# angeladai/sgnn

Measured on AMD Instinct MI355X. Metric: TSDF blocks/sec fwd+bwd (64^3@5% occ, bs32), higher is better.
Workload: dtype f32

## Files before the change

sgnn_amd/csrc/linear.hip:

```cpp
#include "common.h"

#define LIN_MAX_OUT 4
#define LIN_MAX_BLOCKS 512

template <int CIN, int VEC>
__device__ __forceinline__ void load_row(const float *__restrict__ p, float (&v)[CIN]) {
  if constexpr (VEC == 4) {
#pragma unroll
    for (int t = 0; t < CIN / 4; ++t) {
      const float4 q = reinterpret_cast<const float4 *>(p)[t];
      v[4 * t] = q.x; v[4 * t + 1] = q.y; v[4 * t + 2] = q.z; v[4 * t + 3] = q.w;
    }
  } else {
#pragma unroll
    for (int t = 0; t < CIN; ++t) v[t] = p[t];
  }
}

struct LinW {
  const float *w[LIN_MAX_OUT];
  const float *b[LIN_MAX_OUT];
};
struct LinG {
  float *dw[LIN_MAX_OUT];
  float *db[LIN_MAX_OUT];
};

template <int CIN, int COUT>
__global__ __launch_bounds__(256) void k_linear_fwd(const float *__restrict__ x, int64_t n, LinW p,
                                                   float *__restrict__ y, const int64_t *n_dev) {
  __shared__ float ws[COUT * CIN + COUT];
  n = sgnn_dyn_n(n, n_dev);
  for (int e = threadIdx.x; e < COUT * CIN; e += 256) ws[e] = p.w[e / CIN][e % CIN];
  if (threadIdx.x < COUT) ws[COUT * CIN + threadIdx.x] = p.b[threadIdx.x] ? p.b[threadIdx.x][0] : 0.f;
  __syncthreads();
  const int64_t stride = (int64_t)gridDim.x * 256;
  for (int64_t r = (int64_t)blockIdx.x * 256 + threadIdx.x; r < n; r += stride) {
    float v[CIN];
    load_row<CIN, (CIN % 4 == 0) ? 4 : 1>(x + r * CIN, v);
#pragma unroll
    for (int o = 0; o < COUT; ++o) {
      float acc = ws[COUT * CIN + o];
#pragma unroll
      for (int c = 0; c < CIN; ++c) acc = fmaf(v[c], ws[o * CIN + c], acc);
      y[r * COUT + o] = acc;
    }
  }
}

template <int CIN, int COUT>
__global__ __launch_bounds__(256) void k_linear_bwd(const float *__restrict__ x, const float *__restrict__ dy,
                                                   int64_t n, LinW p, float *dx, double *__restrict__ partial,
                                                   const int64_t *n_dev, const float *addend, int64_t ld_add) {
  constexpr int NV = COUT * CIN + COUT;
  n = sgnn_dyn_n(n, n_dev);
  __shared__ float ws[COUT * CIN];
  __shared__ float red[4][NV];
  for (int e = threadIdx.x; e < COUT * CIN; e += 256) ws[e] = p.w[e / CIN][e % CIN];
  __syncthreads();
  float acc[NV];
#pragma unroll
  for (int e = 0; e < NV; ++e) acc[e] = 0.f;
  const int64_t stride = (int64_t)gridDim.x * 256;
  for (int64_t r = (int64_t)blockIdx.x * 256 + threadIdx.x; r < n; r += stride) {
    float v[CIN], g[COUT];
    load_row<CIN, (CIN % 4 == 0) ? 4 : 1>(x + r * CIN, v);
#pragma unroll
    for (int o = 0; o < COUT; ++o) g[o] = dy[r * COUT + o];
#pragma unroll
    for (int o = 0; o < COUT; ++o) {
#pragma unroll
      for (int c = 0; c < CIN; ++c) acc[o * CIN + c] = fmaf(g[o], v[c], acc[o * CIN + c]);
      acc[COUT * CIN + o] += g[o];
    }
    if (dx) {
      float d[CIN];
#pragma unroll
      for (int c = 0; c < CIN; ++c) {
        float t = 0.f;
#pragma unroll
        for (int o = 0; o < COUT; ++o) t = fmaf(g[o], ws[o * CIN + c], t);
        d[c] = t;
      }
      if (addend) {
        float a[CIN];
        load_row<CIN, (CIN % 4 == 0) ? 4 : 1>(addend + r * ld_add, a);
#pragma unroll
        for (int c = 0; c < CIN; ++c) d[c] += a[c];
      }
      if constexpr (CIN % 4 == 0) {
#pragma unroll
        for (int t = 0; t < CIN / 4; ++t)
          reinterpret_cast<float4 *>(dx + r * CIN)[t] = make_float4(d[4 * t], d[4 * t + 1], d[4 * t + 2], d[4 * t + 3]);
      } else {
#pragma unroll
        for (int c = 0; c < CIN; ++c) dx[r * CIN + c] = d[c];
      }
    }
  }
  const int lane = threadIdx.x & 63, wave = threadIdx.x >> 6;
#pragma unroll
  for (int e = 0; e < NV; ++e) {
    float t = acc[e];
#pragma unroll
    for (int d = 32; d > 0; d >>= 1) t += __shfl_xor(t, d);
    if (lane == 0) red[wave][e] = t;
  }
  __syncthreads();
  for (int e = threadIdx.x; e < NV; e += 256)
    partial[(size_t)blockIdx.x * NV + e] = (double)red[0][e] + (double)red[1][e] + (double)red[2][e] + (double)red[3][e];
}

__global__ __launch_bounds__(256) void k_linear_finalize(const double *__restrict__ partial, int nblk, int nv,
                                                        int ncw, int cin, LinG g) {
  __shared__ double sh[256];
  const int e = blockIdx.x;
  double a = 0.0;
  for (int b = threadIdx.x; b < nblk; b += 256) a += partial[(size_t)b * nv + e];
  sh[threadIdx.x] = a;
  __syncthreads();
  for (int d = 128; d > 0; d >>= 1) {
    if (threadIdx.x < d) sh[threadIdx.x] += sh[threadIdx.x + d];
    __syncthreads();
  }
  if (threadIdx.x == 0) {
    if (e < ncw) {
      if (g.dw[e / cin]) g.dw[e / cin][e % cin] = (float)sh[0];
    } else if (g.db[e - ncw]) {
      g.db[e - ncw][0] = (float)sh[0];
    }
  }
}

static int lin_blocks(int64_t n) {
  int64_t b = (n + 255) / 256;
  if (b < 1) b = 1;
  if (b > LIN_MAX_BLOCKS) b = LIN_MAX_BLOCKS;
  return (int)b;
}

SGNN_EXPORT int64_t sgnn_linear_ws_bytes(int64_t n, int cin, int cout) {
  (void)n;
  return (int64_t)LIN_MAX_BLOCKS * (cin * cout + cout) * (int64_t)sizeof(double) + 256;
}

#define LIN_CASES(X) X(16, 1) X(16, 2) X(48, 1) X(48, 2) X(8, 1) X(8, 2) X(32, 1) X(32, 2) X(12, 2) X(4, 1)

static bool lin_shape_ok(int cin, int cout) {
#define X(CI, CO) if (cin == CI && cout == CO) return true;
  LIN_CASES(X)
#undef X
  return false;
}

int sgnn_linear_fwd_rows(const float *x, int64_t n, int cin, const float *const *w, const float *const *b, int cout,
                         float *y, sgnn_stream_t stream, const int64_t *n_dev) {
  SGNN_CHECK_ARG(n >= 0 && cin >= 1 && cout >= 1 && cout <= LIN_MAX_OUT);
  if (!lin_shape_ok(cin, cout)) {
    sgnn_set_error("sgnn_linear_fwd: unsupported head shape %d -> %d", cin, cout);
    return SGNN_EINVAL;
  }
  if (n == 0) return SGNN_OK;
  SGNN_CHECK_ARG(x && w && y);
  LinW p{};
  for (int o = 0; o < cout; ++o) {
    SGNN_CHECK_ARG(w[o]);
    p.w[o] = w[o];
    p.b[o] = b ? b[o] : nullptr;
  }
  hipStream_t s = (hipStream_t)stream;
  const int grid = sgnn_grid_for(n, 256, 2048);
  bool done = false;
#define X(CI, CO)                                                                                   \
  if (!done && cin == CI && cout == CO) {                                                           \
    SGNN_LAUNCH((k_linear_fwd<CI, CO>), dim3(grid), dim3(256), 0, s, x, n, p, y, n_dev);     \
    done = true;                                                                                    \
  }
  LIN_CASES(X)
#undef X
  if (!done) {
    sgnn_set_error("sgnn_linear_fwd: unsupported head shape %d -> %d", cin, cout);
    return SGNN_EINVAL;
  }
  SGNN_CHECK_LAUNCH();
  return SGNN_OK;
}

SGNN_EXPORT int sgnn_linear_fwd(const float *x, int64_t n, int cin, const float *w, const float *bias, int cout,
                                float *y, sgnn_stream_t stream) {
  SGNN_CHECK_ARG(cout >= 1 && cout <= LIN_MAX_OUT && cin >= 1);
  const float *wr[LIN_MAX_OUT] = {}, *br[LIN_MAX_OUT] = {};
  for (int o = 0; o < cout; ++o) {
    wr[o] = w ? w + (size_t)o * cin : nullptr;
    br[o] = bias ? bias + o : nullptr;
  }
  return sgnn_linear_fwd_rows(x, n, cin, wr, br, cout, y, stream);
}

int sgnn_linear_bwd_rows(const float *x, const float *dy, int64_t n, int cin, const float *const *w, int cout,
                         float *dx, float *const *dw, float *const *db, void *ws, int64_t ws_bytes,
                         sgnn_stream_t stream, const int64_t *n_dev, const float *addend, int64_t ld_add) {
  hipStream_t s = (hipStream_t)stream;
  SGNN_CHECK_ARG(n >= 0 && cin >= 1 && cout >= 1 && cout <= LIN_MAX_OUT && w);
  SGNN_CHECK_ARG(!addend || (dx && ld_add >= cin && (cin % 4 != 0 || (ld_add % 4 == 0 && ((uintptr_t)addend & 15) == 0))));
  if (!lin_shape_ok(cin, cout)) {
    sgnn_set_error("sgnn_linear_bwd: unsupported head shape %d -> %d", cin, cout);
    return SGNN_EINVAL;
  }
  if (n == 0) {
    for (int o = 0; o < cout; ++o) {
      if (dw && dw[o]) SGNN_HIP_TRY(hipMemsetAsync(dw[o], 0, (size_t)cin * sizeof(float), s));
      if (db && db[o]) SGNN_HIP_TRY(hipMemsetAsync(db[o], 0, sizeof(float), s));
    }
    return SGNN_OK;
  }
  SGNN_CHECK_ARG(x && dy);
  if (!ws || ws_bytes < sgnn_linear_ws_bytes(n, cin, cout)) {
    sgnn_set_error("sgnn_linear_bwd: workspace too small");
    return SGNN_ENOWS;
  }
  LinW p{};
  LinG g{};
  for (int o = 0; o < cout; ++o) {
    SGNN_CHECK_ARG(w[o]);
    p.w[o] = w[o];
    g.dw[o] = dw ? dw[o] : nullptr;
    g.db[o] = db ? db[o] : nullptr;
  }
  const int nblk = lin_blocks(n);
  const int nv = cin * cout + cout;
  bool done = false;
#define X(CI, CO)                                                                                          \
  if (!done && cin == CI && cout == CO) {                                                                  \
    SGNN_LAUNCH((k_linear_bwd<CI, CO>), dim3(nblk), dim3(256), 0, s, x, dy, n, p, dx, (double *)ws, n_dev, addend, ld_add); \
    done = true;                                                                                           \
  }
  LIN_CASES(X)
#undef X
  if (!done) {
    sgnn_set_error("sgnn_linear_bwd: unsupported head shape %d -> %d", cin, cout);
    return SGNN_EINVAL;
  }
  SGNN_LAUNCH(k_linear_finalize, dim3(nv), dim3(256), 0, s, (const double *)ws, nblk, nv, cin * cout, cin, g);
  SGNN_CHECK_LAUNCH();
  return SGNN_OK;
}

SGNN_EXPORT int sgnn_linear_bwd(const float *x, const float *dy, int64_t n, int cin, const float *w, int cout,
                                float *dx, float *dw, float *dbias, void *ws, int64_t ws_bytes,
                                sgnn_stream_t stream) {
  SGNN_CHECK_ARG(cout >= 1 && cout <= LIN_MAX_OUT && cin >= 1 && w);
  const float *wr[LIN_MAX_OUT] = {};
  float *dwr[LIN_MAX_OUT] = {}, *dbr[LIN_MAX_OUT] = {};
  for (int o = 0; o < cout; ++o) {
    wr[o] = w + (size_t)o * cin;
    dwr[o] = dw ? dw + (size_t)o * cin : nullptr;
    dbr[o] = dbias ? dbias + o : nullptr;
  }
  return sgnn_linear_bwd_rows(x, dy, n, cin, wr, cout, dx, dwr, dbr, ws, ws_bytes, stream);
}
```

sgnn_amd/csrc/loss.hip:

```cpp
#include "common.h"

#define LOSS_MAX_BLOCKS 512
#define UNK_ID_F (-1.0f)
#define UNK_THRESH_U8 2

struct LossArgs {
  const int64_t *locs;
  const float *vals;
  int vstride, occ_col, sdf_col;
  const float *tgt_occ;
  const float *tgt_sdf;
  const float *weights;
  const uint8_t *known;
  int d0, d1, d2;
  int64_t m;
  const int64_t *m_dev;
  int use_log;
  int mask_mode;
};

__device__ __forceinline__ float logt(float v) { return copysignf(logf(fabsf(v) + 1.0f), v) * (v != 0.f); }

__device__ __forceinline__ bool loss_site(const LossArgs &a, int64_t r, float &bce, float &l1, float &dbce, float &dl1) {
  const longlong2 p0 = reinterpret_cast<const longlong2 *>(a.locs)[2 * r];
  const longlong2 p1 = reinterpret_cast<const longlong2 *>(a.locs)[2 * r + 1];
  const int64_t fl = ((p1.y * a.d0 + p0.x) * a.d1 + p0.y) * a.d2 + p1.x;
  const float w = a.weights ? a.weights[fl] : 1.0f;
  float to = 0.f;
  bool keep = true;
  if (a.tgt_occ) to = a.tgt_occ[fl];
  if (a.mask_mode == 1) keep = (to != UNK_ID_F);
  if (a.mask_mode == 2) keep = a.known[fl] < UNK_THRESH_U8;
  if (a.mask_mode == 0 && to == UNK_ID_F) to = 0.f;
  bce = l1 = dbce = dl1 = 0.f;
  if (!keep) return false;
  if (a.occ_col >= 0) {
    const float x = a.vals[r * a.vstride + a.occ_col];
    const float t = fmaxf(to, 0.f);
    bce = w * (fmaxf(x, 0.f) - x * t + log1pf(expf(-fabsf(x))));
    dbce = w * (1.0f / (1.0f + expf(-x)) - t);
  }
  if (a.sdf_col >= 0) {
    const float p = a.vals[r * a.vstride + a.sdf_col];
    const float t = a.tgt_sdf[fl];
    const float d = a.use_log ? (logt(p) - logt(t)) : (p - t);
    l1 = w * fabsf(d);
    const float sg = (d > 0.f) ? 1.f : ((d < 0.f) ? -1.f : 0.f);
    dl1 = w * sg * (a.use_log ? 1.0f / (fabsf(p) + 1.0f) : 1.0f);
  }
  return true;
}

static int loss_blocks(int64_t m) {
  int64_t b = (m + 1023) / 1024;
  if (b < 1) b = 1;
  if (b > LOSS_MAX_BLOCKS) b = LOSS_MAX_BLOCKS;
  return (int)b;
}

static int fill_args(LossArgs &a, const int64_t *locs, const float *vals, int vstride, int occ_col, int sdf_col,
                     const float *tgt_occ, const float *tgt_sdf, const float *weights, const uint8_t *known, int d0,
                     int d1, int d2, int64_t m, int use_log, int mask_mode, const int64_t *m_dev) {
  if (!(m >= 0 && vstride >= 1 && occ_col < vstride && sdf_col < vstride && (occ_col >= 0 || sdf_col >= 0))) return -1;
  if (m > 0 && (!locs || !vals)) return -1;
  if (occ_col >= 0 && !tgt_occ) return -1;
  if (sdf_col >= 0 && !tgt_sdf) return -1;
  if (mask_mode == 1 && !tgt_occ) return -1;
  if (mask_mode == 2 && !known) return -1;
  if (mask_mode < 0 || mask_mode > 2) return -1;
  a = LossArgs{locs, vals, vstride, occ_col, sdf_col, tgt_occ, tgt_sdf, weights, known, d0, d1, d2, m, m_dev, use_log, mask_mode};
  return 0;
}

#define LOSS_MAX_LEVELS 5
struct LossMulti {
  LossArgs a[LOSS_MAX_LEVELS];
  float coef[2 * LOSS_MAX_LEVELS];
  int nblk[LOSS_MAX_LEVELS];
  int n;
};
struct LossOut {
  float *dvals[LOSS_MAX_LEVELS];
};

__global__ __launch_bounds__(256) void k_loss_partial(LossMulti m, double *__restrict__ partial) {
  __shared__ double sh[3][256];
  const int l = blockIdx.y;
  const LossArgs &a = m.a[l];
  if ((int)blockIdx.x >= m.nblk[l]) return;
  double s[3] = {0.0, 0.0, 0.0};
  const int64_t stride = (int64_t)m.nblk[l] * 256;
  const int64_t rows = sgnn_dyn_n(a.m, a.m_dev);
  for (int64_t r = (int64_t)blockIdx.x * 256 + threadIdx.x; r < rows; r += stride) {
    float bce, l1, db, dl;
    if (loss_site(a, r, bce, l1, db, dl)) {
      s[0] += (double)bce;
      s[1] += (double)l1;
      s[2] += 1.0;
    }
  }
  sgnn_block_sum256(sh, s);
  if (threadIdx.x < 3) partial[((size_t)l * LOSS_MAX_BLOCKS + blockIdx.x) * 3 + threadIdx.x] = sh[threadIdx.x][0];
}

__global__ __launch_bounds__(256) void k_loss_finalize(const double *__restrict__ partial, LossMulti m,
                                                      double *__restrict__ sums, float *__restrict__ out2s,
                                                      float *__restrict__ total, float *__restrict__ cur) {
  __shared__ double sh[3][256];
  for (int l = 0; l < m.n; ++l) {
    double s[3] = {0.0, 0.0, 0.0};
    for (int b = threadIdx.x; b < m.nblk[l]; b += 256)
      for (int c = 0; c < 3; ++c) s[c] += partial[((size_t)l * LOSS_MAX_BLOCKS + b) * 3 + c];
    sgnn_block_sum256(sh, s);
    if (threadIdx.x == 0) {
      sums[3 * l + 0] = sh[0][0];
      sums[3 * l + 1] = sh[1][0];
      sums[3 * l + 2] = sh[2][0];
      const bool empty = m.a[l].m_dev && *m.a[l].m_dev <= 0;
      out2s[2 * l] = empty ? 0.f : (float)(sh[0][0] / sh[2][0]);
      out2s[2 * l + 1] = empty ? 0.f : (float)(sh[1][0] / sh[2][0]);
    }
    __syncthreads();
  }
  if (threadIdx.x == 0) {
    float t = 0.f;
    for (int i = 0; i < 2 * m.n; ++i)
      if (m.coef[i] != 0.f) t += m.coef[i] * out2s[i];
    *total = t;
    for (int l = 0; l < m.n; ++l)
      cur[l] = (m.coef[2 * l] != 0.f ? out2s[2 * l] : 0.f) + (m.coef[2 * l + 1] != 0.f ? out2s[2 * l + 1] : 0.f);
  }
}

__global__ __launch_bounds__(256) void k_loss_bwd(LossMulti m, const double *__restrict__ sums,
                                                 const float *__restrict__ g, LossOut o) {
  const int l = blockIdx.y;
  const LossArgs &a = m.a[l];
  float *dvals = o.dvals[l];
  const double kept = sums[3 * l + 2];
  const float g0 = (float)((double)(g[0] * m.coef[2 * l]) / kept), g1 = (float)((double)(g[0] * m.coef[2 * l + 1]) / kept);
  const int64_t stride = (int64_t)gridDim.x * 256;
  const int64_t rows = sgnn_dyn_n(a.m, a.m_dev);
  for (int64_t r = (int64_t)blockIdx.x * 256 + threadIdx.x; r < rows; r += stride) {
    float bce, l1, db, dl;
    const bool keep = loss_site(a, r, bce, l1, db, dl);
    for (int c = 0; c < a.vstride; ++c) {
      float v = 0.f;
      if (keep && c == a.occ_col) v = g0 * db;
      if (keep && c == a.sdf_col) v = g1 * dl;
      dvals[r * a.vstride + c] = v;
    }
  }
}

SGNN_EXPORT int64_t sgnn_loss_multi_ws_bytes(void) {
  return (int64_t)LOSS_MAX_LEVELS * LOSS_MAX_BLOCKS * 3 * sizeof(double) + 64;
}

static int fill_multi(LossMulti &m, const int64_t *levels, int n, const float *coef) {
  if (n < 1 || n > LOSS_MAX_LEVELS || !levels || !coef) return -1;
  m.n = n;
  for (int l = 0; l < n; ++l) {
    const int64_t *v = levels + 16 * l;
    if (fill_args(m.a[l], (const int64_t *)(uintptr_t)v[0], (const float *)(uintptr_t)v[1], (int)v[2], (int)v[3], (int)v[4],
                  (const float *)(uintptr_t)v[5], (const float *)(uintptr_t)v[6], (const float *)(uintptr_t)v[7],
                  (const uint8_t *)(uintptr_t)v[8], (int)v[9], (int)v[10], (int)v[11], v[12], (int)v[13], (int)v[14],
                  (const int64_t *)(uintptr_t)v[15]) != 0)
      return -1;
    m.nblk[l] = loss_blocks(v[12]);
    m.coef[2 * l] = coef[2 * l];
    m.coef[2 * l + 1] = coef[2 * l + 1];
  }
  return 0;
}

SGNN_EXPORT int sgnn_loss_levels_fwd(const int64_t *levels, int n, const float *coef_host, double *sums, float *out2s,
                                     float *total, float *cur, void *ws, int64_t ws_bytes, sgnn_stream_t stream) {
  LossMulti m{};
  SGNN_CHECK_ARG(fill_multi(m, levels, n, coef_host) == 0);
  SGNN_CHECK_ARG(sums && out2s && total && cur);
  if (!ws || ws_bytes < sgnn_loss_multi_ws_bytes()) {
    sgnn_set_error("sgnn_loss_levels_fwd: workspace too small");
    return SGNN_ENOWS;
  }
  int gx = 1;
  for (int l = 0; l < n; ++l) gx = m.nblk[l] > gx ? m.nblk[l] : gx;
  hipStream_t s = (hipStream_t)stream;
  SGNN_LAUNCH(k_loss_partial, dim3(gx, n), dim3(256), 0, s, m, (double *)ws);
  SGNN_LAUNCH(k_loss_finalize, dim3(1), dim3(256), 0, s, (const double *)ws, m, sums, out2s, total, cur);
  SGNN_CHECK_LAUNCH();
  return SGNN_OK;
}

SGNN_EXPORT int sgnn_loss_levels_bwd(const int64_t *levels, int n, const float *coef_host, const double *sums,
                                     const float *g, void *const *dvals, sgnn_stream_t stream) {
  LossMulti m{};
  SGNN_CHECK_ARG(fill_multi(m, levels, n, coef_host) == 0);
  SGNN_CHECK_ARG(sums && g && dvals);
  LossOut o{};
  int64_t mmax = 1;
  for (int l = 0; l < n; ++l) {
    SGNN_CHECK_ARG(dvals[l] || m.a[l].m == 0);
    o.dvals[l] = (float *)dvals[l];
    mmax = m.a[l].m > mmax ? m.a[l].m : mmax;
  }
  SGNN_LAUNCH(k_loss_bwd, dim3(sgnn_grid_for(mmax, 256, 2048), n), dim3(256), 0, (hipStream_t)stream, m, sums, g, o);
  SGNN_CHECK_LAUNCH();
  return SGNN_OK;
}

__device__ __forceinline__ float clamp_sdf(float v, float trunc) { return v != v ? v : fminf(fmaxf(v, -trunc), trunc); }

__global__ __launch_bounds__(256) void k_targets_fine(const float *__restrict__ sdf, const uint8_t *__restrict__ known,
                                                     int64_t total, float trunc, int masking, float wmg,
                                                     float *__restrict__ tsdf, float *__restrict__ hier_last,
                                                     float *__restrict__ occ, float *__restrict__ w) {
  const int64_t stride = (int64_t)gridDim.x * 256;
  for (int64_t i = (int64_t)blockIdx.x * 256 + threadIdx.x; i < total; i += stride) {
    const float t = clamp_sdf(sdf[i], trunc);
    tsdf[i] = t;
    hier_last[i] = t;
    float o = fabsf(t) < trunc ? 1.f : 0.f;
    if (masking && known[i] >= UNK_THRESH_U8) o = UNK_ID_F;
    occ[i] = o;
    if (w) w[i] = (fabsf(o) <= trunc) ? wmg : 1.f;
  }
}

__global__ __launch_bounds__(256) void k_targets_sites(const int64_t *__restrict__ locs, int64_t n, int batch, int d0,
                                                      int d1, int d2, float *__restrict__ w, const int64_t *n_dev) {
  n = sgnn_dyn_n(n, n_dev);
  const int64_t stride = (int64_t)gridDim.x * 256;
  for (int64_t r = (int64_t)blockIdx.x * 256 + threadIdx.x; r < n; r += stride) {
    const longlong2 p0 = reinterpret_cast<const longlong2 *>(locs)[2 * r];
    const longlong2 p1 = reinterpret_cast<const longlong2 *>(locs)[2 * r + 1];
    if (p0.x < 0 || p0.x >= d0 || p0.y < 0 || p0.y >= d1 || p1.x < 0 || p1.x >= d2 || p1.y < 0 || p1.y >= batch) continue;
    w[((p1.y * d0 + p0.x) * d1 + p0.y) * d2 + p1.x] = 1.f;
  }
}

struct CoarseArgs {
  const float *occ_f, *w_f;
  const float *hier_in[3];
  float *occ[3], *w[3], *hier[3];
  int batch, d0, d1, d2;
  float trunc;
  int nlev;
};

__global__ __launch_bounds__(256) void k_targets_coarse(CoarseArgs a) {
  const int lane = threadIdx.x & 63;
  const int lz = lane >> 4, ly = (lane >> 2) & 3, lx = lane & 3;
  const int c0 = a.d0 >> 1, c1 = a.d1 >> 1, c2 = a.d2 >> 1;
  const int b0 = (c0 + 3) >> 2, b1 = (c1 + 3) >> 2, b2 = (c2 + 3) >> 2;
  const int64_t bricks = (int64_t)a.batch * b0 * b1 * b2;
  const int64_t wave0 = (int64_t)blockIdx.x * 4 + (threadIdx.x >> 6), nwaves = (int64_t)gridDim.x * 4;
  for (int64_t br = wave0; br < bricks; br += nwaves) {
    int64_t t = br;
    const int bx = (int)(t % b2); t /= b2;
    const int by = (int)(t % b1); t /= b1;
    const int bz = (int)(t % b0);
    const int b = (int)(t / b0);
    const int z = bz * 4 + lz, y = by * 4 + ly, x = bx * 4 + lx;
    const bool in = z < c0 && y < c1 && x < c2;
    float m = -INFINITY;
    if (in) {
      const float *p = a.occ_f + (((int64_t)b * a.d0 + 2 * z) * a.d1 + 2 * y) * a.d2 + 2 * x;
#pragma unroll
      for (int dz = 0; dz < 2; ++dz)
#pragma unroll
        for (int dy = 0; dy < 2; ++dy) {
          const float2 v = *reinterpret_cast<const float2 *>(p + ((int64_t)dz * a.d1 + dy) * a.d2);
          m = fmaxf(m, fmaxf(v.x, v.y));
        }
      const int64_t o = (((int64_t)b * c0 + z) * c1 + y) * c2 + x;
      a.occ[0][o] = m;
      if (a.w[0]) a.w[0][o] = a.w_f[(((int64_t)b * a.d0 + 2 * z) * a.d1 + 2 * y) * a.d2 + 2 * x];
      a.hier[0][o] = clamp_sdf(a.hier_in[0][o], a.trunc);
    }
    if (a.nlev >= 2) {
      m = fmaxf(m, __shfl_xor(m, 1));
      m = fmaxf(m, __shfl_xor(m, 4));
      m = fmaxf(m, __shfl_xor(m, 16));
      const int e0 = c0 >> 1, e1 = c1 >> 1, e2 = c2 >> 1;
      const int zz = z >> 1, yy = y >> 1, xx = x >> 1;
      if (((lz | ly | lx) & 1) == 0 && zz < e0 && yy < e1 && xx < e2) {
        const int64_t o = (((int64_t)b * e0 + zz) * e1 + yy) * e2 + xx;
        a.occ[1][o] = m;
        if (a.w[1]) a.w[1][o] = a.w_f[(((int64_t)b * a.d0 + 4 * zz) * a.d1 + 4 * yy) * a.d2 + 4 * xx];
        a.hier[1][o] = clamp_sdf(a.hier_in[1][o], a.trunc);
      }
      if (a.nlev >= 3) {
        m = fmaxf(m, __shfl_xor(m, 2));
        m = fmaxf(m, __shfl_xor(m, 8));
        m = fmaxf(m, __shfl_xor(m, 32));
        const int f0 = e0 >> 1, f1 = e1 >> 1, f2 = e2 >> 1;
        if (lane == 0 && bz < f0 && by < f1 && bx < f2) {
          const int64_t o = (((int64_t)b * f0 + bz) * f1 + by) * f2 + bx;
          a.occ[2][o] = m;
          if (a.w[2]) a.w[2][o] = a.w_f[(((int64_t)b * a.d0 + 8 * bz) * a.d1 + 8 * by) * a.d2 + 8 * bx];
          a.hier[2][o] = clamp_sdf(a.hier_in[2][o], a.trunc);
        }
      }
    }
  }
}

SGNN_EXPORT int sgnn_loss_targets(const float *sdf, const uint8_t *known, const int64_t *input_locs, int64_t n_locs,
                                  const int64_t *n_locs_dev, int batch, int d0, int d1, int d2, float trunc, int masking, float weight_missing_geo,
                                  int ncoarse, void *const *hier_in, float *tsdf, float *hier_last, float *occ_last,
                                  float *w_last, void *const *occ, void *const *w, void *const *hier,
                                  sgnn_stream_t stream) {
  hipStream_t s = (hipStream_t)stream;
  SGNN_CHECK_ARG(batch >= 0 && d0 >= 1 && d1 >= 1 && d2 >= 1 && ncoarse >= 0 && ncoarse <= 3 && n_locs >= 0);
  SGNN_CHECK_ARG((d0 % (1 << ncoarse)) == 0 && (d1 % (1 << ncoarse)) == 0 && (d2 % (1 << ncoarse)) == 0);
  const int64_t total = (int64_t)batch * d0 * d1 * d2;
  if (total == 0) return SGNN_OK;
  SGNN_CHECK_ARG(sdf && tsdf && hier_last && occ_last && (!masking || known) && (!w_last || n_locs == 0 || input_locs));
  SGNN_CHECK_ARG(ncoarse == 0 || (hier_in && occ && hier && (!w_last || w)));
  SGNN_LAUNCH(k_targets_fine, dim3(sgnn_grid_for(total, 256, 4096)), dim3(256), 0, s, sdf, known, total, trunc,
                     masking, weight_missing_geo, tsdf, hier_last, occ_last, w_last);
  if (w_last && n_locs > 0)
    SGNN_LAUNCH(k_targets_sites, dim3(sgnn_grid_for(n_locs, 256, 4096)), dim3(256), 0, s, input_locs, n_locs,
                       batch, d0, d1, d2, w_last, n_locs_dev);
  if (ncoarse > 0) {
    CoarseArgs a{};
    a.occ_f = occ_last;
    a.w_f = w_last;
    for (int k = 0; k < ncoarse; ++k) {
      SGNN_CHECK_ARG(hier_in[k] && occ[k] && hier[k] && (!w_last || w[k]));
      a.hier_in[k] = (const float *)hier_in[k];
      a.occ[k] = (float *)occ[k];
      a.w[k] = w_last ? (float *)w[k] : nullptr;
      a.hier[k] = (float *)hier[k];
    }
    a.batch = batch; a.d0 = d0; a.d1 = d1; a.d2 = d2; a.trunc = trunc; a.nlev = ncoarse;
    const int64_t bricks = (int64_t)batch * ((d0 / 2 + 3) / 4) * ((d1 / 2 + 3) / 4) * ((d2 / 2 + 3) / 4);
    SGNN_LAUNCH(k_targets_coarse, dim3(sgnn_grid_for(bricks, 4, 8192)), dim3(256), 0, s, a);
  }
  SGNN_CHECK_LAUNCH();
  return SGNN_OK;
}
```

Baseline: 5712.

## Fuse dense target pyramid kernels and restructure loss and linear backward loops

The fine and coarse target kernels become one tiled kernel that computes fine targets and all coarse occupancy/weight/hier levels in a single pass, using shuffles and shared memory, so occ_f is no longer re-read. The site kernel now also sets coarse weights at aligned positions. The loss kernels batch several rows in flight, use float2 loads and stores for two-column rows, and run a parallel wave-based finalize. Linear backward splits the dx computation into its own element-parallel loop with multiple loads in flight, at the cost of reading dy twice. These changes target launch count, redundant memory traffic and memory latency, but add complexity in coarse-weight semantics and edge handling.

```diff
diff --git a/sgnn_amd/csrc/linear.hip b/sgnn_amd/csrc/linear.hip
--- a/sgnn_amd/csrc/linear.hip
+++ b/sgnn_amd/csrc/linear.hip
@@ -2,6 +2,7 @@
 
 #define LIN_MAX_OUT 4
 #define LIN_MAX_BLOCKS 512
+#define LIN_DX_IN_FLIGHT 4
 
 template <int CIN, int VEC>
 __device__ __forceinline__ void load_row(const float *__restrict__ p, float (&v)[CIN]) {
@@ -62,6 +63,43 @@
 #pragma unroll
   for (int e = 0; e < NV; ++e) acc[e] = 0.f;
   const int64_t stride = (int64_t)gridDim.x * 256;
+  if (dx) {
+    constexpr int W = (CIN % 4 == 0) ? 4 : 1, Q = CIN / W;
+    const int64_t pieces = n * Q;
+    for (int64_t e0 = (int64_t)blockIdx.x * 256 + threadIdx.x; e0 < pieces; e0 += LIN_DX_IN_FLIGHT * stride) {
+      float g[LIN_DX_IN_FLIGHT][COUT], a[LIN_DX_IN_FLIGHT][W];
+#pragma unroll
+      for (int k = 0; k < LIN_DX_IN_FLIGHT; ++k) {
+        const int64_t e = e0 + k * stride;
+        if (e < pieces) {
+          const int64_t r = e / Q;
+          const int q = (int)(e % Q);
+#pragma unroll
+          for (int o = 0; o < COUT; ++o) g[k][o] = dy[r * COUT + o];
+          if (addend) load_row<W, W>(addend + r * ld_add + q * W, a[k]);
+        }
+      }
+#pragma unroll
+      for (int k = 0; k < LIN_DX_IN_FLIGHT; ++k) {
+        const int64_t e = e0 + k * stride;
+        if (e >= pieces) break;
+        const int q = (int)(e % Q);
+        float d[W];
+#pragma unroll
+        for (int c = 0; c < W; ++c) {
+          float t = 0.f;
+#pragma unroll
+          for (int o = 0; o < COUT; ++o) t = fmaf(g[k][o], ws[o * CIN + q * W + c], t);
+          d[c] = addend ? t + a[k][c] : t;
+        }
+        if constexpr (W == 4) {
+          reinterpret_cast<float4 *>(dx)[e] = make_float4(d[0], d[1], d[2], d[3]);
+        } else {
+          dx[e] = d[0];
+        }
+      }
+    }
+  }
   for (int64_t r = (int64_t)blockIdx.x * 256 + threadIdx.x; r < n; r += stride) {
     float v[CIN], g[COUT];
     load_row<CIN, (CIN % 4 == 0) ? 4 : 1>(x + r * CIN, v);
@@ -72,30 +110,6 @@
 #pragma unroll
       for (int c = 0; c < CIN; ++c) acc[o * CIN + c] = fmaf(g[o], v[c], acc[o * CIN + c]);
       acc[COUT * CIN + o] += g[o];
-    }
-    if (dx) {
-      float d[CIN];
-#pragma unroll
-      for (int c = 0; c < CIN; ++c) {
-        float t = 0.f;
-#pragma unroll
-        for (int o = 0; o < COUT; ++o) t = fmaf(g[o], ws[o * CIN + c], t);
-        d[c] = t;
-      }
-      if (addend) {
-        float a[CIN];
-        load_row<CIN, (CIN % 4 == 0) ? 4 : 1>(addend + r * ld_add, a);
-#pragma unroll
-        for (int c = 0; c < CIN; ++c) d[c] += a[c];
-      }
-      if constexpr (CIN % 4 == 0) {
-#pragma unroll
-        for (int t = 0; t < CIN / 4; ++t)
-          reinterpret_cast<float4 *>(dx + r * CIN)[t] = make_float4(d[4 * t], d[4 * t + 1], d[4 * t + 2], d[4 * t + 3]);
-      } else {
-#pragma unroll
-        for (int c = 0; c < CIN; ++c) dx[r * CIN + c] = d[c];
-      }
     }
   }
   const int lane = threadIdx.x & 63, wave = threadIdx.x >> 6;
@@ -202,6 +216,7 @@
                          sgnn_stream_t stream, const int64_t *n_dev, const float *addend, int64_t ld_add) {
   hipStream_t s = (hipStream_t)stream;
   SGNN_CHECK_ARG(n >= 0 && cin >= 1 && cout >= 1 && cout <= LIN_MAX_OUT && w);
+  SGNN_CHECK_ARG(!dx || dx != x);
   SGNN_CHECK_ARG(!addend || (dx && ld_add >= cin && (cin % 4 != 0 || (ld_add % 4 == 0 && ((uintptr_t)addend & 15) == 0))));
   if (!lin_shape_ok(cin, cout)) {
     sgnn_set_error("sgnn_linear_bwd: unsupported head shape %d -> %d", cin, cout);
diff --git a/sgnn_amd/csrc/loss.hip b/sgnn_amd/csrc/loss.hip
--- a/sgnn_amd/csrc/loss.hip
+++ b/sgnn_amd/csrc/loss.hip
@@ -21,28 +21,52 @@
 
 __device__ __forceinline__ float logt(float v) { return copysignf(logf(fabsf(v) + 1.0f), v) * (v != 0.f); }
 
-__device__ __forceinline__ bool loss_site(const LossArgs &a, int64_t r, float &bce, float &l1, float &dbce, float &dl1) {
+struct LossSite {
+  float w, to, x, p, t;
+  bool keep;
+};
+
+__device__ __forceinline__ bool loss_pair_rows(const LossArgs &a, const void *rows) {
+  return a.vstride == 2 && a.occ_col == 0 && a.sdf_col == 1 && ((uintptr_t)rows & 7) == 0;
+}
+
+__device__ __forceinline__ LossSite loss_load(const LossArgs &a, int64_t r, bool pair) {
   const longlong2 p0 = reinterpret_cast<const longlong2 *>(a.locs)[2 * r];
   const longlong2 p1 = reinterpret_cast<const longlong2 *>(a.locs)[2 * r + 1];
   const int64_t fl = ((p1.y * a.d0 + p0.x) * a.d1 + p0.y) * a.d2 + p1.x;
-  const float w = a.weights ? a.weights[fl] : 1.0f;
-  float to = 0.f;
-  bool keep = true;
-  if (a.tgt_occ) to = a.tgt_occ[fl];
-  if (a.mask_mode == 1) keep = (to != UNK_ID_F);
-  if (a.mask_mode == 2) keep = a.known[fl] < UNK_THRESH_U8;
-  if (a.mask_mode == 0 && to == UNK_ID_F) to = 0.f;
+  LossSite s;
+  s.w = a.weights ? a.weights[fl] : 1.0f;
+  s.to = a.tgt_occ ? a.tgt_occ[fl] : 0.f;
+  s.keep = true;
+  if (a.mask_mode == 1) s.keep = (s.to != UNK_ID_F);
+  if (a.mask_mode == 2) s.keep = a.known[fl] < UNK_THRESH_U8;
+  if (a.mask_mode == 0 && s.to == UNK_ID_F) s.to = 0.f;
+  s.x = s.p = s.t = 0.f;
+  if (pair) {
+    const float2 v = reinterpret_cast<const float2 *>(a.vals)[r];
+    s.x = v.x;
+    s.p = v.y;
+  } else {
+    if (a.occ_col >= 0) s.x = a.vals[r * a.vstride + a.occ_col];
+    if (a.sdf_col >= 0) s.p = a.vals[r * a.vstride + a.sdf_col];
+  }
+  if (a.sdf_col >= 0) s.t = a.tgt_sdf[fl];
+  return s;
+}
+
+__device__ __forceinline__ bool loss_eval(const LossArgs &a, const LossSite &s, float &bce, float &l1, float &dbce, float &dl1) {
   bce = l1 = dbce = dl1 = 0.f;
-  if (!keep) return false;
+  if (!s.keep) return false;
+  const float w = s.w;
   if (a.occ_col >= 0) {
-    const float x = a.vals[r * a.vstride + a.occ_col];
-    const float t = fmaxf(to, 0.f);
+    const float x = s.x;
+    const float t = fmaxf(s.to, 0.f);
     bce = w * (fmaxf(x, 0.f) - x * t + log1pf(expf(-fabsf(x))));
     dbce = w * (1.0f / (1.0f + expf(-x)) - t);
   }
   if (a.sdf_col >= 0) {
-    const float p = a.vals[r * a.vstride + a.sdf_col];
-    const float t = a.tgt_sdf[fl];
+    const float p = s.p;
+    const float t = s.t;
     const float d = a.use_log ? (logt(p) - logt(t)) : (p - t);
     l1 = w * fabsf(d);
     const float sg = (d > 0.f) ? 1.f : ((d < 0.f) ? -1.f : 0.f);
@@ -83,6 +107,7 @@
   float *dvals[LOSS_MAX_LEVELS];
 };
 
+#define LOSS_ROWS_IN_FLIGHT 4
 __global__ __launch_bounds__(256) void k_loss_partial(LossMulti m, double *__restrict__ partial) {
   __shared__ double sh[3][256];
   const int l = blockIdx.y;
@@ -91,38 +116,57 @@
   double s[3] = {0.0, 0.0, 0.0};
   const int64_t stride = (int64_t)m.nblk[l] * 256;
   const int64_t rows = sgnn_dyn_n(a.m, a.m_dev);
-  for (int64_t r = (int64_t)blockIdx.x * 256 + threadIdx.x; r < rows; r += stride) {
-    float bce, l1, db, dl;
-    if (loss_site(a, r, bce, l1, db, dl)) {
-      s[0] += (double)bce;
-      s[1] += (double)l1;
-      s[2] += 1.0;
+  const bool pair = loss_pair_rows(a, a.vals);
+  for (int64_t r0 = (int64_t)blockIdx.x * 256 + threadIdx.x; r0 < rows; r0 += LOSS_ROWS_IN_FLIGHT * stride) {
+    LossSite site[LOSS_ROWS_IN_FLIGHT];
+#pragma unroll
+    for (int k = 0; k < LOSS_ROWS_IN_FLIGHT; ++k)
+      if (r0 + k * stride < rows) site[k] = loss_load(a, r0 + k * stride, pair);
+#pragma unroll
+    for (int k = 0; k < LOSS_ROWS_IN_FLIGHT; ++k) {
+      float bce, l1, db, dl;
+      if (r0 + k * stride < rows && loss_eval(a, site[k], bce, l1, db, dl)) {
+        s[0] += (double)bce;
+        s[1] += (double)l1;
+        s[2] += 1.0;
+      }
     }
   }
   sgnn_block_sum256(sh, s);
   if (threadIdx.x < 3) partial[((size_t)l * LOSS_MAX_BLOCKS + blockIdx.x) * 3 + threadIdx.x] = sh[threadIdx.x][0];
 }
 
-__global__ __launch_bounds__(256) void k_loss_finalize(const double *__restrict__ partial, LossMulti m,
-                                                      double *__restrict__ sums, float *__restrict__ out2s,
-                                                      float *__restrict__ total, float *__restrict__ cur) {
-  __shared__ double sh[3][256];
-  for (int l = 0; l < m.n; ++l) {
-    double s[3] = {0.0, 0.0, 0.0};
-    for (int b = threadIdx.x; b < m.nblk[l]; b += 256)
-      for (int c = 0; c < 3; ++c) s[c] += partial[((size_t)l * LOSS_MAX_BLOCKS + b) * 3 + c];
-    sgnn_block_sum256(sh, s);
-    if (threadIdx.x == 0) {
-      sums[3 * l + 0] = sh[0][0];
-      sums[3 * l + 1] = sh[1][0];
-      sums[3 * l + 2] = sh[2][0];
+__global__ __launch_bounds__(1024) void k_loss_finalize(const double *__restrict__ partial, LossMulti m,
+                                                       double *__restrict__ sums, float *__restrict__ out2s,
+                                                       float *__restrict__ total, float *__restrict__ cur) {
+  __shared__ double sh[3 * LOSS_MAX_LEVELS];
+  const int lane = threadIdx.x & 63, q = threadIdx.x >> 6;
+  if (q < 3 * m.n) {
+    const int l = q / 3, c = q % 3;
+    double v[4];
+#pragma unroll
+    for (int j = 0; j < 4; ++j) {
+      double t = 0.0;
+      for (int b = lane + 64 * j; b < m.nblk[l]; b += 256) t += partial[((size_t)l * LOSS_MAX_BLOCKS + b) * 3 + c];
+      v[j] = t;
+    }
+    v[0] += v[2];
+    v[1] += v[3];
+    double t = v[0] + v[1];
+#pragma unroll
+    for (int d = 32; d > 0; d >>= 1) t += __shfl_down(t, d);
+    if (lane == 0) sh[q] = t;
+  }
+  __syncthreads();
+  if (threadIdx.x == 0) {
+    for (int l = 0; l < m.n; ++l) {
+      sums[3 * l + 0] = sh[3 * l + 0];
+      sums[3 * l + 1] = sh[3 * l + 1];
+      sums[3 * l + 2] = sh[3 * l + 2];
       const bool empty = m.a[l].m_dev && *m.a[l].m_dev <= 0;
-      out2s[2 * l] = empty ? 0.f : (float)(sh[0][0] / sh[2][0]);
-      out2s[2 * l + 1] = empty ? 0.f : (float)(sh[1][0] / sh[2][0]);
-    }
-    __syncthreads();
-  }
-  if (threadIdx.x == 0) {
+      out2s[2 * l] = empty ? 0.f : (float)(sh[3 * l + 0] / sh[3 * l + 2]);
+      out2s[2 * l + 1] = empty ? 0.f : (float)(sh[3 * l + 1] / sh[3 * l + 2]);
+    }
     float t = 0.f;
     for (int i = 0; i < 2 * m.n; ++i)
       if (m.coef[i] != 0.f) t += m.coef[i] * out2s[i];
@@ -137,13 +181,20 @@
   const int l = blockIdx.y;
   const LossArgs &a = m.a[l];
   float *dvals = o.dvals[l];
+  const int64_t stride = (int64_t)gridDim.x * 256;
+  const int64_t rows = sgnn_dyn_n(a.m, a.m_dev);
+  if ((int64_t)blockIdx.x * 256 >= rows) return;
   const double kept = sums[3 * l + 2];
   const float g0 = (float)((double)(g[0] * m.coef[2 * l]) / kept), g1 = (float)((double)(g[0] * m.coef[2 * l + 1]) / kept);
-  const int64_t stride = (int64_t)gridDim.x * 256;
-  const int64_t rows = sgnn_dyn_n(a.m, a.m_dev);
+  const bool pair = loss_pair_rows(a, a.vals) && ((uintptr_t)dvals & 7) == 0;
   for (int64_t r = (int64_t)blockIdx.x * 256 + threadIdx.x; r < rows; r += stride) {
     float bce, l1, db, dl;
-    const bool keep = loss_site(a, r, bce, l1, db, dl);
+    const LossSite site = loss_load(a, r, pair);
+    const bool keep = loss_eval(a, site, bce, l1, db, dl);
+    if (pair) {
+      reinterpret_cast<float2 *>(dvals)[r] = keep ? make_float2(g0 * db, g1 * dl) : make_float2(0.f, 0.f);
+      continue;
+    }
     for (int c = 0; c < a.vstride; ++c) {
       float v = 0.f;
       if (keep && c == a.occ_col) v = g0 * db;
@@ -187,7 +238,7 @@
   for (int l = 0; l < n; ++l) gx = m.nblk[l] > gx ? m.nblk[l] : gx;
   hipStream_t s = (hipStream_t)stream;
   SGNN_LAUNCH(k_loss_partial, dim3(gx, n), dim3(256), 0, s, m, (double *)ws);
-  SGNN_LAUNCH(k_loss_finalize, dim3(1), dim3(256), 0, s, (const double *)ws, m, sums, out2s, total, cur);
+  SGNN_LAUNCH(k_loss_finalize, dim3(1), dim3(1024), 0, s, (const double *)ws, m, sums, out2s, total, cur);
   SGNN_CHECK_LAUNCH();
   return SGNN_OK;
 }
@@ -211,24 +262,146 @@
 
 __device__ __forceinline__ float clamp_sdf(float v, float trunc) { return v != v ? v : fminf(fmaxf(v, -trunc), trunc); }
 
-__global__ __launch_bounds__(256) void k_targets_fine(const float *__restrict__ sdf, const uint8_t *__restrict__ known,
-                                                     int64_t total, float trunc, int masking, float wmg,
-                                                     float *__restrict__ tsdf, float *__restrict__ hier_last,
-                                                     float *__restrict__ occ, float *__restrict__ w) {
-  const int64_t stride = (int64_t)gridDim.x * 256;
-  for (int64_t i = (int64_t)blockIdx.x * 256 + threadIdx.x; i < total; i += stride) {
-    const float t = clamp_sdf(sdf[i], trunc);
-    tsdf[i] = t;
-    hier_last[i] = t;
-    float o = fabsf(t) < trunc ? 1.f : 0.f;
-    if (masking && known[i] >= UNK_THRESH_U8) o = UNK_ID_F;
-    occ[i] = o;
-    if (w) w[i] = (fabsf(o) <= trunc) ? wmg : 1.f;
-  }
-}
+struct TargetArgs {
+  const float *sdf;
+  const uint8_t *known;
+  float *tsdf, *hier_last, *occ_f, *w_f;
+  const float *hier_in[3];
+  float *occ[3], *w[3], *hier[3];
+  int batch, d0, d1, d2;
+  float trunc, wmg;
+  int masking;
+  int nlev;
+};
+
+template <bool V4>
+__global__ __launch_bounds__(256) void k_targets_dense(TargetArgs a) {
+  __shared__ float sh_m[4][4], sh_w[4];
+  const int t = threadIdx.x, wave = t >> 6;
+  const int xq = t & 7, zl = (t >> 3) & 3, yp = (wave & 1) * 2 + ((t >> 5) & 1);
+  const int n2 = (a.d2 + 31) >> 5, n1 = (a.d1 + 7) >> 3, n0 = (a.d0 + 7) >> 3;
+  int64_t tile = blockIdx.x;
+  const int tx = (int)(tile % n2); tile /= n2;
+  const int ty = (int)(tile % n1); tile /= n1;
+  const int tz = (int)(tile % n0);
+  const int b = (int)(tile / n0);
+  const int Z = tz * 8 + (wave >> 1) * 4 + zl, Y = ty * 8 + 2 * yp, X = tx * 32 + 4 * xq;
+  float om[2][4];
+  float w00 = 0.f, w02 = 0.f;
+#pragma unroll
+  for (int j = 0; j < 2; ++j) {
+    const bool rowin = Z < a.d0 && Y + j < a.d1;
+    const int64_t base = (((int64_t)b * a.d0 + Z) * a.d1 + Y + j) * a.d2 + X;
+    float s[4] = {0.f, 0.f, 0.f, 0.f};
+    uint8_t kn[4] = {0, 0, 0, 0};
+    bool in[4];
+#pragma unroll
+    for (int i = 0; i < 4; ++i) in[i] = rowin && X + i < a.d2;
+    if (V4) {
+      if (in[0]) {
+        const float4 q = *reinterpret_cast<const float4 *>(a.sdf + base);
+        s[0] = q.x; s[1] = q.y; s[2] = q.z; s[3] = q.w;
+        if (a.masking) {
+          const uchar4 k = *reinterpret_cast<const uchar4 *>(a.known + base);
+          kn[0] = k.x; kn[1] = k.y; kn[2] = k.z; kn[3] = k.w;
+        }
+      }
+    } else {
+#pragma unroll
+      for (int i = 0; i < 4; ++i)
+        if (in[i]) {
+          s[i] = a.sdf[base + i];
+          if (a.masking) kn[i] = a.known[base + i];
+        }
+    }
+    float ts[4], o[4], wv[4];
+#pragma unroll
+    for (int i = 0; i < 4; ++i) {
+      ts[i] = clamp_sdf(s[i], a.trunc);
+      o[i] = fabsf(ts[i]) < a.trunc ? 1.f : 0.f;
+      if (a.masking && kn[i] >= UNK_THRESH_U8) o[i] = UNK_ID_F;
+      wv[i] = (fabsf(o[i]) <= a.trunc) ? a.wmg : 1.f;
+      om[j][i] = in[i] ? o[i] : -INFINITY;
+    }
+    if (j == 0) { w00 = wv[0]; w02 = wv[2]; }
+    if (V4) {
+      if (in[0]) {
+        const float4 tq = make_float4(ts[0], ts[1], ts[2], ts[3]);
+        *reinterpret_cast<float4 *>(a.tsdf + base) = tq;
+        *reinterpret_cast<float4 *>(a.hier_last + base) = tq;
+        *reinterpret_cast<float4 *>(a.occ_f + base) = make_float4(o[0], o[1], o[2], o[3]);
+        if (a.w_f) *reinterpret_cast<float4 *>(a.w_f + base) = make_float4(wv[0], wv[1], wv[2], wv[3]);
+      }
+    } else {
+#pragma unroll
+      for (int i = 0; i < 4; ++i)
+        if (in[i]) {
+          a.tsdf[base + i] = ts[i];
+          a.hier_last[base + i] = ts[i];
+          a.occ_f[base + i] = o[i];
+          if (a.w_f) a.w_f[base + i] = wv[i];
+        }
+    }
+  }
+  if (a.nlev < 1) return;
+  const bool in0 = Z < a.d0 && Y < a.d1 && X < a.d2, in2 = Z < a.d0 && Y < a.d1 && X + 2 < a.d2;
+  float m0 = fmaxf(fmaxf(om[0][0], om[0][1]), fmaxf(om[1][0], om[1][1]));
+  float m1 = fmaxf(fmaxf(om[0][2], om[0][3]), fmaxf(om[1][2], om[1][3]));
+  m0 = fmaxf(m0, __shfl_xor(m0, 8));
+  m1 = fmaxf(m1, __shfl_xor(m1, 8));
+  if ((zl & 1) == 0) {
+    const int c0 = a.d0 >> 1, c1 = a.d1 >> 1, c2 = a.d2 >> 1;
+    const int64_t o = (((int64_t)b * c0 + (Z >> 1)) * c1 + (Y >> 1)) * c2 + (X >> 1);
+    if (in0) {
+      a.occ[0][o] = m0;
+      if (a.w[0]) a.w[0][o] = w00;
+      a.hier[0][o] = clamp_sdf(a.hier_in[0][o], a.trunc);
+    }
+    if (in2) {
+      a.occ[0][o + 1] = m1;
+      if (a.w[0]) a.w[0][o + 1] = w02;
+      a.hier[0][o + 1] = clamp_sdf(a.hier_in[0][o + 1], a.trunc);
+    }
+  }
+  if (a.nlev < 2) return;
+  float m = fmaxf(m0, m1);
+  m = fmaxf(m, __shfl_xor(m, 32));
+  m = fmaxf(m, __shfl_xor(m, 16));
+  const bool corner = zl == 0 && (yp & 1) == 0;
+  if (corner && in0) {
+    const int e0 = a.d0 >> 2, e1 = a.d1 >> 2, e2 = a.d2 >> 2;
+    const int64_t o = (((int64_t)b * e0 + (Z >> 2)) * e1 + (Y >> 2)) * e2 + (X >> 2);
+    a.occ[1][o] = m;
+    if (a.w[1]) a.w[1][o] = w00;
+    a.hier[1][o] = clamp_sdf(a.hier_in[1][o], a.trunc);
+  }
+  if (a.nlev < 3) return;
+  m = fmaxf(m, __shfl_xor(m, 1));
+  if (corner && (xq & 1) == 0) {
+    sh_m[wave][xq >> 1] = m;
+    if (wave == 0) sh_w[xq >> 1] = w00;
+  }
+  __syncthreads();
+  if (t < 4) {
+    const int z8 = tz * 8, y8 = ty * 8, x8 = tx * 32 + 8 * t;
+    if (z8 < a.d0 && y8 < a.d1 && x8 < a.d2) {
+      const int f0 = a.d0 >> 3, f1 = a.d1 >> 3, f2 = a.d2 >> 3;
+      const int64_t o = (((int64_t)b * f0 + tz) * f1 + ty) * f2 + (x8 >> 3);
+      a.occ[2][o] = fmaxf(fmaxf(sh_m[0][t], sh_m[1][t]), fmaxf(sh_m[2][t], sh_m[3][t]));
+      if (a.w[2]) a.w[2][o] = sh_w[t];
+      a.hier[2][o] = clamp_sdf(a.hier_in[2][o], a.trunc);
+    }
+  }
+}
+
+struct SiteW {
+  float *w[3];
+  int nlev;
+};
 
 __global__ __launch_bounds__(256) void k_targets_sites(const int64_t *__restrict__ locs, int64_t n, int batch, int d0,
-                                                      int d1, int d2, float *__restrict__ w, const int64_t *n_dev) {
+                                                      int d1, int d2, float *__restrict__ w, SiteW cw,
+                                                      const int64_t *n_dev) {
   n = sgnn_dyn_n(n, n_dev);
   const int64_t stride = (int64_t)gridDim.x * 256;
   for (int64_t r = (int64_t)blockIdx.x * 256 + threadIdx.x; r < n; r += stride) {
@@ -236,72 +409,9 @@
     const longlong2 p1 = reinterpret_cast<const longlong2 *>(locs)[2 * r + 1];
     if (p0.x < 0 || p0.x >= d0 || p0.y < 0 || p0.y >= d1 || p1.x < 0 || p1.x >= d2 || p1.y < 0 || p1.y >= batch) continue;
     w[((p1.y * d0 + p0.x) * d1 + p0.y) * d2 + p1.x] = 1.f;
-  }
-}
-
-struct CoarseArgs {
-  const float *occ_f, *w_f;
-  const float *hier_in[3];
-  float *occ[3], *w[3], *hier[3];
-  int batch, d0, d1, d2;
-  float trunc;
-  int nlev;
-};
-
-__global__ __launch_bounds__(256) void k_targets_coarse(CoarseArgs a) {
-  const int lane = threadIdx.x & 63;
-  const int lz = lane >> 4, ly = (lane >> 2) & 3, lx = lane & 3;
-  const int c0 = a.d0 >> 1, c1 = a.d1 >> 1, c2 = a.d2 >> 1;
-  const int b0 = (c0 + 3) >> 2, b1 = (c1 + 3) >> 2, b2 = (c2 + 3) >> 2;
-  const int64_t bricks = (int64_t)a.batch * b0 * b1 * b2;
-  const int64_t wave0 = (int64_t)blockIdx.x * 4 + (threadIdx.x >> 6), nwaves = (int64_t)gridDim.x * 4;
-  for (int64_t br = wave0; br < bricks; br += nwaves) {
-    int64_t t = br;
-    const int bx = (int)(t % b2); t /= b2;
-    const int by = (int)(t % b1); t /= b1;
-    const int bz = (int)(t % b0);
-    const int b = (int)(t / b0);
-    const int z = bz * 4 + lz, y = by * 4 + ly, x = bx * 4 + lx;
-    const bool in = z < c0 && y < c1 && x < c2;
-    float m = -INFINITY;
-    if (in) {
-      const float *p = a.occ_f + (((int64_t)b * a.d0 + 2 * z) * a.d1 + 2 * y) * a.d2 + 2 * x;
-#pragma unroll
-      for (int dz = 0; dz < 2; ++dz)
-#pragma unroll
-        for (int dy = 0; dy < 2; ++dy) {
-          const float2 v = *reinterpret_cast<const float2 *>(p + ((int64_t)dz * a.d1 + dy) * a.d2);
-          m = fmaxf(m, fmaxf(v.x, v.y));
-        }
-      const int64_t o = (((int64_t)b * c0 + z) * c1 + y) * c2 + x;
-      a.occ[0][o] = m;
-      if (a.w[0]) a.w[0][o] = a.w_f[(((int64_t)b * a.d0 + 2 * z) * a.d1 + 2 * y) * a.d2 + 2 * x];
-      a.hier[0][o] = clamp_sdf(a.hier_in[0][o], a.trunc);
-    }
-    if (a.nlev >= 2) {
-      m = fmaxf(m, __shfl_xor(m, 1));
-      m = fmaxf(m, __shfl_xor(m, 4));
-      m = fmaxf(m, __shfl_xor(m, 16));
-      const int e0 = c0 >> 1, e1 = c1 >> 1, e2 = c2 >> 1;
-      const int zz = z >> 1, yy = y >> 1, xx = x >> 1;
-      if (((lz | ly | lx) & 1) == 0 && zz < e0 && yy < e1 && xx < e2) {
-        const int64_t o = (((int64_t)b * e0 + zz) * e1 + yy) * e2 + xx;
-        a.occ[1][o] = m;
-        if (a.w[1]) a.w[1][o] = a.w_f[(((int64_t)b * a.d0 + 4 * zz) * a.d1 + 4 * yy) * a.d2 + 4 * xx];
-        a.hier[1][o] = clamp_sdf(a.hier_in[1][o], a.trunc);
-      }
-      if (a.nlev >= 3) {
-        m = fmaxf(m, __shfl_xor(m, 2));
-        m = fmaxf(m, __shfl_xor(m, 8));
-        m = fmaxf(m, __shfl_xor(m, 32));
-        const int f0 = e0 >> 1, f1 = e1 >> 1, f2 = e2 >> 1;
-        if (lane == 0 && bz < f0 && by < f1 && bx < f2) {
-          const int64_t o = (((int64_t)b * f0 + bz) * f1 + by) * f2 + bx;
-          a.occ[2][o] = m;
-          if (a.w[2]) a.w[2][o] = a.w_f[(((int64_t)b * a.d0 + 8 * bz) * a.d1 + 8 * by) * a.d2 + 8 * bx];
-          a.hier[2][o] = clamp_sdf(a.hier_in[2][o], a.trunc);
-        }
-      }
+    for (int k = 1; k <= cw.nlev; ++k) {
+      if (((p0.x | p0.y | p1.x) & ((1 << k) - 1)) != 0) break;
+      cw.w[k - 1][((p1.y * (d0 >> k) + (p0.x >> k)) * (d1 >> k) + (p0.y >> k)) * (d2 >> k) + (p1.x >> k)] = 1.f;
     }
   }
 }
@@ -318,26 +428,29 @@
   if (total == 0) return SGNN_OK;
   SGNN_CHECK_ARG(sdf && tsdf && hier_last && occ_last && (!masking || known) && (!w_last || n_locs == 0 || input_locs));
   SGNN_CHECK_ARG(ncoarse == 0 || (hier_in && occ && hier && (!w_last || w)));
-  SGNN_LAUNCH(k_targets_fine, dim3(sgnn_grid_for(total, 256, 4096)), dim3(256), 0, s, sdf, known, total, trunc,
-                     masking, weight_missing_geo, tsdf, hier_last, occ_last, w_last);
+  TargetArgs a{};
+  SiteW cw{};
+  a.sdf = sdf; a.known = masking ? known : nullptr;
+  a.tsdf = tsdf; a.hier_last = hier_last; a.occ_f = occ_last; a.w_f = w_last;
+  for (int k = 0; k < ncoarse; ++k) {
+    SGNN_CHECK_ARG(hier_in[k] && occ[k] && hier[k] && (!w_last || w[k]));
+    a.hier_in[k] = (const float *)hier_in[k];
+    a.occ[k] = (float *)occ[k];
+    a.w[k] = cw.w[k] = w_last ? (float *)w[k] : nullptr;
+    a.hier[k] = (float *)hier[k];
+  }
+  a.batch = batch; a.d0 = d0; a.d1 = d1; a.d2 = d2; a.trunc = trunc; a.wmg = weight_missing_geo;
+  a.masking = masking; a.nlev = cw.nlev = ncoarse;
+  const int64_t tiles = (int64_t)batch * ((d0 + 7) / 8) * ((d1 + 7) / 8) * ((d2 + 31) / 32);
+  SGNN_CHECK_ARG(tiles <= INT32_MAX);
+  const uintptr_t align = (uintptr_t)sdf | (uintptr_t)tsdf | (uintptr_t)hier_last | (uintptr_t)occ_last | (uintptr_t)w_last;
+  if (d2 % 4 == 0 && (align & 15) == 0 && (!masking || ((uintptr_t)known & 3) == 0))
+    SGNN_LAUNCH(k_targets_dense<true>, dim3((unsigned)tiles), dim3(256), 0, s, a);
+  else
+    SGNN_LAUNCH(k_targets_dense<false>, dim3((unsigned)tiles), dim3(256), 0, s, a);
   if (w_last && n_locs > 0)
     SGNN_LAUNCH(k_targets_sites, dim3(sgnn_grid_for(n_locs, 256, 4096)), dim3(256), 0, s, input_locs, n_locs,
-                       batch, d0, d1, d2, w_last, n_locs_dev);
-  if (ncoarse > 0) {
-    CoarseArgs a{};
-    a.occ_f = occ_last;
-    a.w_f = w_last;
-    for (int k = 0; k < ncoarse; ++k) {
-      SGNN_CHECK_ARG(hier_in[k] && occ[k] && hier[k] && (!w_last || w[k]));
-      a.hier_in[k] = (const float *)hier_in[k];
-      a.occ[k] = (float *)occ[k];
-      a.w[k] = w_last ? (float *)w[k] : nullptr;
-      a.hier[k] = (float *)hier[k];
-    }
-    a.batch = batch; a.d0 = d0; a.d1 = d1; a.d2 = d2; a.trunc = trunc; a.nlev = ncoarse;
-    const int64_t bricks = (int64_t)batch * ((d0 / 2 + 3) / 4) * ((d1 / 2 + 3) / 4) * ((d2 / 2 + 3) / 4);
-    SGNN_LAUNCH(k_targets_coarse, dim3(sgnn_grid_for(bricks, 4, 8192)), dim3(256), 0, s, a);
-  }
+                       batch, d0, d1, d2, w_last, cw, n_locs_dev);
   SGNN_CHECK_LAUNCH();
   return SGNN_OK;
 }
```

New measurement: 5693 (median of 2 runs). No clear change (-0.3%).
